# Sachin-A/TraceWeaver

Hardware: AMD Instinct MI355X
Metric: spans/sec reconstructed + assignment accuracy vs ground truth (higher is better)
Workload: dtype int64 timestamps, f64 scores; 1 GPU; media_microservices shape (6 services, E in {1,1,1,1,2,4}), 100000 requests/service x 16 replicas per GPU, concurrency 1.6, two-pass reconstruction, device mixture refit; spans_per_gpu=25600000, spans_total=25600000, parallelism=units sharded, 1 rank(s), backend none

## Files before the change

### traceweaver_amd/csrc/tw_engine.hip

```cpp
#include <algorithm>
#include <chrono>
#include <cmath>
#include <cstdio>
#include <cstdlib>
#include <cstring>
#include <functional>
#include <string>
#include <type_traits>
#include <vector>

#include <hip/hip_runtime.h>
#include <rocprim/rocprim.hpp>

#include "traceweaver_amd.h"
#include "tw_kernels.h"
#include "tw_fit.h"
#include "tw_eval.h"
#include "tw_skip.h"
#include "tw_load.h"
#include "tw_baselines.h"
#include "tw_stitch.h"
#include "tw_attr.h"
#include "tw_conf.h"
#include "tw_dist.h"
// ... 45 lines not shown

}

struct tw_engine {
    int device = 0;
    hipStream_t stream = nullptr;
    hipStream_t cls_stream[kMaxEp + 1] = {};
    hipEvent_t cls_ev[kMaxEp + 2] = {};
    hipStream_t sel_stream[3] = {};
    hipStream_t sel_stream2[3] = {};
    int64_t select_fork_min = 0;
    hipEvent_t prep_ev = nullptr;
    hipEvent_t post_fork[kMaxEp + 1] = {}, post_join[kMaxEp + 1][3] = {}, post_done[kMaxEp + 1] = {};
    hipEvent_t tile_ev[kMaxEp + 1] = {};
    hipStream_t cls_stream2[kMaxEp + 1] = {};
    hipEvent_t stretch_ev[kMaxEp + 1][kEnumStretches] = {}, stretch_done[kMaxEp + 1] = {};
    int enum_stretches = 1, stretch_min_tiles = 2048;
    int heavy_grid = 4096, select_grid = 0;
    int debug_lists = 0;
    int32_t first_lists[3][kMaxEp + 1] = {};
    hipEvent_t gate_ev = nullptr;
    int tile_gate = 0;
    int stage_min_tiles = 1024;
    int32_t *rank_in = nullptr, *rank_out = nullptr;
    bool class_params = false;
    int prio_min_e = 0, prio_high = 0;
    bool prio_any = false;
    int pipeline = 1;
    std::string err;
    int state = ST_EMPTY;
    int tile = kTile;
    int tile_threads = 2;
    int tile_single = 1;
    int tile_single_threads = 1;
    int coop = kCoop;
    std::vector<UnitDev> units;
    std::vector<TileDev> tiles;
    std::vector<int64_t> gs_off_h;
    std::vector<void*> allocs;
    void* arena = nullptr;
    size_t arena_cap = 0;
    bool arena_open = false;
    std::vector<std::pair<std::function<void(void*)>, size_t>> arena_req;
    Dev P{};
    int64_t n_ie = 0, n_gp = 0, n_slots = 0, n_gaps = 0;
    PairVI* agg_pair = nullptr;
    int32_t *agg_i32 = nullptr, *agg_i32b = nullptr;
    uint32_t *seg_in = nullptr, *seg_out = nullptr;
    int n_seg_out = 0;
    void* sort_tmp = nullptr;
    size_t sort_tmp_bytes = 0;
    double* mix_p_dev = nullptr;
    int32_t* mix_n_dev = nullptr;
    double* mix_c_dev = nullptr;
    double* gaps_sorted = nullptr;
    double* fit_models = nullptr;
    double* fit_uval = nullptr;
    int32_t *fit_ustart = nullptr, *fit_row_n = nullptr, *fit_row_uniq = nullptr;
    double* fit_centres = nullptr;
    double *fit_tape = nullptr, *fit_tape100 = nullptr;
    int64_t* fit_tape_off = nullptr;
    int64_t fit_tape_cap = 0;
    bool fit_runs_pending = false;
    bool fit_prepared = false;
    int tile_sub_max = 8;
    int32_t hard_pass1[kMaxEp + 1] = {};
    int8_t wide_pass1[kMaxEp + 1] = {};
    int32_t split_pass1[kMaxEp + 1] = {};
    int lean_pool = 512;
    bool pass1_done = false;
    std::vector<int32_t> fit_max_n;
    bool fit_max_n_valid = false;
    Mt19937 fit_rng;
    uint32_t fit_seed = 0;
    int32_t* slot_unit = nullptr;
    int32_t* tile_ids = nullptr;
    int32_t* ctr = nullptr;
    int64_t ctr_round_ints = 0, ctr_pass_ints = 0;
    int32_t tile_cls_off[kMaxEp + 2] = {};
    uint32_t *seg_gap = nullptr, *seg_gap_end = nullptr, *seg_gap_dst = nullptr;
    unsigned long long *comp_a = nullptr, *comp_b = nullptr;
    int64_t comp_cap = 0, n_gap_scored = 0;
    int32_t *truth = nullptr, *in_trace = nullptr;
    uint8_t* trace_bad = nullptr;
    unsigned long long* eval_counts = nullptr;
    int64_t n_traces = 0, trace_cap = 0;
    uint8_t* slot_scored = nullptr;
    int64_t n_gap_rows = 0;
    unsigned long long* key_acc = nullptr;
    double fit_ms = 0.0;
    int rounds = 0;
    bool skip_mode = false;
    SkipUnitDev* skip_units = nullptr;
    int32_t* skip_perm = nullptr; int64_t* skip_tw = nullptr; int32_t* skip_pool = nullptr; double* skip_dist = nullptr; long long* skip_fetch = nullptr;
    int64_t skip_fetch_n = 0;
    int64_t *orig_is = nullptr, *orig_ie = nullptr, *orig_os = nullptr, *orig_oe = nullptr;
    int32_t *orig_truth = nullptr, *orig_trace = nullptr;
    bool scaled_upload = false;
    hipEvent_t ev[EV_COUNT] = {};
    double ms[6] = {0, 0, 0, 0, 0, 0};
    StitchDev S{};
    int32_t* given_parent = nullptr;
    bool rows_set = false, parents_given = false, stitched = false;
    int64_t rows_cap = 0, st_trees = 0;
    int stitched_pass = -1;
    bool stitched_truth = false;
    AttrDev A{};
    bool groups_set = false, attributed = false;
    int64_t groups_cap = 0, attr_rows_cap = 0;
    ConfDev C{};
    int64_t conf_rows_cap = 0;
    DistDev D{};
// ... 183 lines not shown
    switch (code) {
        case TW_ERR_WINDOW_WIDTH: return "an incoming span has more candidate spans at one endpoint than the candidate bitmap holds";
        case TW_ERR_WINDOW_SIZE: return "a window holds more than TW_MAX_WINDOW incoming spans";
        case TW_ERR_NAN_PARAMS: return "a parameter block holds a single sample (std = NaN); the reference aborts here (n_in % 100 == 1)";
        case TW_ERR_SKIP_PARAMS: return "skip mode: the scorer needs a (mean, std) pair that BuildDistributions did not produce (the reference raises KeyError)";
        case TW_ERR_SKIP_REFERENCE_RAISES: return "skip mode: the reference raises on this input (all endpoints skipped, or a score tie compared through a skip span)";
        case TW_ERR_ARG: return "skip mode: a request starts before the first time window";
        default: return "kernel reported an error";
    }
}

template <class Tr>
int run_scan(tw_engine* e, const TileSet& S, hipStream_t st, typename Tr::T* agg) {
    const Dev& P = e->P;
    hipLaunchKernelGGL((k_scan_local<Tr>), dim3(S.n), dim3(e->tile), 0, st, P, S, agg);
    hipLaunchKernelGGL((k_scan_spine<Tr>), dim3(P.n_units), dim3(e->coop), 0, st, P, S, agg);
    hipLaunchKernelGGL((k_scan_fix<Tr>), dim3(S.n), dim3(e->tile), 0, st, P, S, agg);
    HIPCHK(hipGetLastError());
    return TW_OK;
}

TileSet all_tiles_host(const tw_engine* e) { return TileSet{nullptr, 0, e->P.n_tiles, 0}; }
TileSet class_tiles(const tw_engine* e, int E) { return TileSet{e->tile_ids + e->tile_cls_off[E], e->tile_cls_off[E], e->tile_cls_off[E + 1] - e->tile_cls_off[E], E}; }

int sort_ends(tw_engine* e, const TileSet& S, hipStream_t st) {
    const Dev& P = e->P;
    const dim3 tiles(S.n), tb(e->tile);
    hipLaunchKernelGGL(k_rank_ends, tiles, tb, 0, st, P, S, e->rank_in, e->rank_out);
    hipLaunchKernelGGL(k_place_ends, tiles, tb, 0, st, P, S, (const int32_t*)e->rank_in, (const int32_t*)e->rank_out);
    HIPCHK(hipGetLastError());
    return TW_OK;
}

int64_t part_extra(int cls, int64_t n_cls) {
    if (n_cls <= 0) return 0;
    static const int deep = env_int("TW_PART_BUDGET_DEEP", 2), shallow = env_int("TW_PART_BUDGET_SHALLOW", 0);
    if (cls <= 1) return 64;
    const int mult = cls >= 5 ? deep : shallow;
    return (mult > 0 ? n_cls * mult : n_cls / 8) + 64;
}

template <int E>
void launch_enumerate(tw_engine* e, int pass, int mode, const int32_t* listed) {
    const int nt = e->tile_cls_off[E + 1] - e->tile_cls_off[E];
    if (nt == 0) return;
    const int n_narrow = listed != nullptr ? listed[E] : -1, n_wide = listed != nullptr ? listed[kMaxEp + 1 + E] : ((pass == 2 && mode == 0 && e->wide_pass1[E] == 0) ? 0 : -1);
    if (n_narrow == 0 && n_wide == 0) return;
    hipStream_t st = e->cls_stream[E];
    (void)hipStreamWaitEvent(st, e->cls_ev[0], 0);
    if (mode == 0 && e->gate_ev != nullptr) (void)hipStreamWaitEvent(st, e->gate_ev, 0);
    const Dev& P = e->P;
    const dim3 hb(std::min(e->coop, kHeavyThreads));
    const int pool = E > 4 ? 2048 : (E > 1 ? kPairPoolPerEp * E : 1);
    const size_t pool_bytes = sizeof(double) * (size_t)pool;
    const size_t lean_bytes = sizeof(double) * (size_t)(2 * kMaxEp * kNarrow + e->lean_pool), lean_bytes_w = sizeof(double) * (size_t)(2 * kMaxEp * 64 * kCandWords + e->lean_pool);
    const bool lean = E >= P.lean_min_e && !e->skip_mode;
    const int cap = P.heavy_in_off[E + 1] - P.heavy_in_off[E];
    auto grid_for = [&](int known, int most) { return std::max(std::min(((known >= 0 ? known : cap) + kWorkChunk - 1) / kWorkChunk, most), 1); };
    auto narrow = [&](int part, int g) {
        if (lean) hipLaunchKernelGGL((k_enumerate_lean<kNarrow>), dim3(g), hb, lean_bytes, st, P, pass, mode, part, e->lean_pool, E, E);
        else hipLaunchKernelGGL((k_enumerate_heavy<E, kNarrow>), dim3(g), hb, pool_bytes, st, P, pass, mode, part, pool);
    };
    auto wide = [&](int part, int g) {
        if (lean) hipLaunchKernelGGL((k_enumerate_lean<64 * kCandWords>), dim3(g), hb, lean_bytes_w, st, P, pass, mode, part, e->lean_pool, E, E);
        else hipLaunchKernelGGL((k_enumerate_heavy<E, 64 * kCandWords>), dim3(g), hb, pool_bytes, st, P, pass, mode, part, pool);
    };
    bool stretched = false;
    if (mode == 0 && pass == 1 && e->class_params) {
        const TileSet S = class_tiles(e, E);
        (void)sort_ends(e, S, st);
        const int64_t total = e->n_gp;
        hipLaunchKernelGGL(k_block_params, dim3((unsigned)((total + 255) / 256)), dim3(256), 0, st, P, total, E);
    }
    if (mode == 0) {
        const bool single = E == 1 && e->tile_single != 0;
        const dim3 tile_block(e->tile >= 64 ? e->tile * (single ? e->tile_single_threads : e->tile_threads) : e->tile);
        int sub = 1;
        while (sub < e->tile_sub_max && nt * sub < 512 && (e->tile / (sub * 2)) * (sub * 2) == e->tile && e->tile / (sub * 2) >= 8) sub *= 2;
        const int ns = (!lean && !e->skip_mode && !(E >= 3 && E >= P.defer_min_e) && e->cls_stream2[E] != nullptr)
                           ? std::max(std::min(e->enum_stretches, nt / e->stretch_min_tiles), 1) : 1;
        stretched = ns > 1;
        for (int j = 0; j < ns; j++) {
            const int t0 = (int)((int64_t)nt * j / ns), t1 = (int)((int64_t)nt * (j + 1) / ns);
            const int32_t* ids = e->tile_ids + e->tile_cls_off[E] + t0;
            const bool sub_tile = e->tile == kTile && e->tile / sub == kSubTileSpans;
            if constexpr (E == 1) {
                if (single && sub_tile) hipLaunchKernelGGL((k_enumerate_tile<1, kSubTileSpans, true>), dim3((t1 - t0) * sub), tile_block, 0, st, P, pass, ids, t1 - t0, sub);
                else if (single) hipLaunchKernelGGL((k_enumerate_tile<1, kTile, true>), dim3((t1 - t0) * sub), tile_block, 0, st, P, pass, ids, t1 - t0, sub);
            }
            if (!single && sub_tile)
                hipLaunchKernelGGL((k_enumerate_tile<E, kSubTileSpans>), dim3((t1 - t0) * sub), tile_block, 0, st, P, pass, ids, t1 - t0, sub);
            else if (!single)
                hipLaunchKernelGGL((k_enumerate_tile<E>), dim3((t1 - t0) * sub), tile_block, 0, st, P, pass, ids, t1 - t0, sub);
            if (ns > 1) {
                hipLaunchKernelGGL(k_enum_snapshot, dim3(1), dim3(1), 0, st, P, E, j + 1);
                if (j + 1 < ns) {
                    hipStream_t s2 = e->cls_stream2[E];
                    (void)hipEventRecord(e->stretch_ev[E][j], st);
                    (void)hipStreamWaitEvent(s2, e->stretch_ev[E][j], 0);
                    hipLaunchKernelGGL((k_enumerate_heavy<E, kNarrow>), dim3(grid_for(-1, e->heavy_grid)), hb, pool_bytes, s2, P, pass, mode, (j + 1) << 8, pool);
                } else {
                    hipLaunchKernelGGL((k_enumerate_heavy<E, kNarrow>), dim3(grid_for(-1, e->heavy_grid)), hb, pool_bytes, st, P, pass, mode, (j + 1) << 8, pool);
                    (void)hipEventRecord(e->stretch_done[E], e->cls_stream2[E]);
                    (void)hipStreamWaitEvent(st, e->stretch_done[E], 0);
                }
// ... 187 lines not shown
    }
    const int bx = (int)std::min<int64_t>(std::max<int64_t>(4096 / nseg, 1), packed / nseg / 1024 + 1);
    const dim3 grid((unsigned)bx, (unsigned)std::min(nseg, 1024)), block(flat_threads(e));
    hipLaunchKernelGGL(k_rows_pack, grid, block, 0, e->stream, (const unsigned long long*)keys, seg_begin, seg_end, dst_off, nseg,
                       (int)begin_bit, (int)kb, e->comp_a);
    TWCHK(rocprim_call(e, [&](void* tmp, size_t& bytes) { return rocprim::radix_sort_keys(tmp, bytes, e->comp_a, e->comp_b, (size_t)packed, 0u, kb + segbits, e->stream); }));
    hipLaunchKernelGGL(k_rows_unpack, grid, block, 0, e->stream, (const unsigned long long*)e->comp_b, seg_begin, seg_end, dst_off, nseg,
                       (int)begin_bit, (int)kb, fixed, (unsigned long long*)out);
    HIPCHK(hipGetLastError());
    return TW_OK;
}

int run_pass(tw_engine* e, int pass) {
    const Dev& P = e->P;
    const dim3 tiles(P.n_tiles), tb(e->tile);
    const auto host_t0 = std::chrono::steady_clock::now();
    HIPCHK(hipEventRecord(e->ev[EV_BEGIN], e->stream));
    HIPCHK(hipMemsetAsync(e->ctr, 0, sizeof(int32_t) * (size_t)e->ctr_pass_ints, e->stream));
#ifdef TW_PROFILE
    HIPCHK(hipMemsetAsync(P.prof + 5, 0, sizeof(unsigned long long) * 3, e->stream));
    HIPCHK(hipMemsetAsync(P.prof + 10, 0, sizeof(unsigned long long) * 3, e->stream));
#endif
    int n_cls = 0;
    for (int E = 1; E <= kMaxEp; E++) n_cls += e->tile_cls_off[E + 1] > e->tile_cls_off[E] ? 1 : 0;
    const bool staged = !e->skip_mode && e->pipeline != 0 && P.n_tiles >= (int64_t)e->stage_min_tiles * std::max(n_cls, 1);
    e->class_params = false;
    if (pass == 1 && !e->skip_mode) {
        HIPCHK(hipMemsetAsync(e->rank_in, 0, sizeof(int32_t) * (size_t)std::max<int64_t>(P.n_in_total, 1), e->stream));
        HIPCHK(hipMemsetAsync(e->rank_out, 0, sizeof(int32_t) * (size_t)std::max<int64_t>(P.n_out_total, 1), e->stream));
        if (staged) e->class_params = true;
        else {
            int rc = sort_ends(e, all_tiles_host(e), e->stream);
            if (rc != TW_OK) return rc;
            const int64_t total = e->n_gp;
            hipLaunchKernelGGL(k_block_params, dim3((unsigned)((total + 255) / 256)), dim3(256), 0, e->stream, P, total, 0);
        }
    }
    if (e->skip_mode) {
        const int64_t total = e->n_gp;
        hipLaunchKernelGGL(k_neutral_params, dim3((unsigned)((total + 255) / 256)), dim3(256), 0, e->stream, P.gparam, total);
    }
    HIPCHK(hipEventRecord(e->ev[EV_PARAMS], e->stream));
    HIPCHK(hipEventRecord(e->ev[EV_ENUM0], e->stream));
    const auto host_t1 = std::chrono::steady_clock::now();
    {
        int rc = launch_enumerate_all(e, pass, 0, nullptr, staged, [&]() -> int {
            if (pass == 1) { int rs = run_scan<ScanMaxEnd>(e, all_tiles_host(e), e->stream, e->agg_pair); if (rs != TW_OK) return rs; }
            if (e->skip_mode) { HIPCHK(hipEventRecord(e->prep_ev, e->stream)); return TW_OK; }
            HIPCHK(hipMemsetAsync(P.w_conf, 0, sizeof(int32_t) * (size_t)P.n_in_total, e->stream));
            HIPCHK(hipMemsetAsync(P.gone_valid, 0, (size_t)P.n_in_total, e->stream));
            HIPCHK(hipMemsetAsync(P.w_dirty, 0, (size_t)P.n_in_total, e->stream));
            HIPCHK(hipMemsetAsync(P.owner, 0x7f, sizeof(int32_t) * std::max<int64_t>(P.n_out_total, 1), e->stream));
            HIPCHK(hipEventRecord(e->prep_ev, e->stream));
            return TW_OK;
        });
        if (rc != TW_OK) return rc;
    }
    e->host_ms[0] = std::chrono::duration<double, std::milli>(std::chrono::steady_clock::now() - host_t1).count();
    if (pass == 1 && !staged) {
        int rc = launch_windows(e, all_tiles_host(e), e->stream);
        if (rc != TW_OK) return rc;
    }
    if (!staged) HIPCHK(hipEventRecord(e->ev[EV_WIN], e->stream));
    if (e->skip_mode) {
        HIPCHK(hipMemsetAsync(P.owner, 0x7f, sizeof(int32_t) * std::max<int64_t>(P.n_out_total, 1), e->stream));
        HIPCHK(hipMemsetAsync(e->skip_fetch, 0, sizeof(long long) * (size_t)std::max<int64_t>(e->skip_fetch_n, 1), e->stream));
        HIPCHK(hipMemsetAsync(P.w_dirty, 0, (size_t)P.n_in_total, e->stream));
        hipLaunchKernelGGL(k_skip_walk, dim3(P.n_units), dim3(std::min(e->coop, 64)), 0, e->stream, P, (const SkipUnitDev*)e->skip_units);
// ... 181 lines not shown
        hipLaunchKernelGGL(k_load_local, dim3(side == 0 ? grid_in : grid_out), dim3(block), 0, e->stream, perm, row, (const uint32_t*)(side == 0 ? e->seg_in : e->seg_out), n);
        HIPCHK(hipGetLastError());
        int32_t* host = side == 0 ? in_perm : out_perm;
        if (host != nullptr) HIPCHK(hipMemcpyAsync(host, perm, sizeof(uint32_t) * n, hipMemcpyDeviceToHost, e->stream));
        HIPCHK(hipStreamSynchronize(e->stream));
    }
    hipLaunchKernelGGL(k_load_retruth, dim3(P.n_tiles), dim3(e->tile), 0, e->stream, L, (const int32_t*)pos_in, (const int32_t*)pos_out, e->truth,
                       has_trace ? e->in_trace : nullptr);
    HIPCHK(hipGetLastError());
    for (int u = 0; u < P.n_units; u++) {
        UnitDev& U = e->units[(size_t)u];
        U.tscale = std::ldexp(1.0, -kmax_h[(size_t)u]);
        U.float_time = 1;
        if (unit_time_scale != nullptr) unit_time_scale[u] = U.tscale;
    }
    HIPCHK(hipMemcpyAsync(const_cast<UnitDev*>(P.units), e->units.data(), sizeof(UnitDev) * e->units.size(), hipMemcpyHostToDevice, e->stream));
    HIPCHK(hipStreamSynchronize(e->stream));
    e->state = ST_LOADED; e->pass1_done = false;
    drop_batch_order(e);
    for (int E = 0; E <= kMaxEp; E++) { e->wide_pass1[E] = -1; e->hard_pass1[E] = -1; e->split_pass1[E] = -1; }
    return TW_OK;
}

extern "C" {

int tw_create(int device_id, tw_engine** out) {
    if (out == nullptr) return TW_ERR_ARG;
    *out = nullptr;
    tw_engine* e = new tw_engine();
    e->device = device_id;
    e->tile = std::min(std::max(env_int("TW_TILE", kTile), 1), kTile);
    e->tile_threads = std::min(std::max(env_int("TW_TILE_THREADS", 2), 1), 4);
    e->tile_single = env_int("TW_TILE_SINGLE", 1);
    e->tile_single_threads = std::min(std::max(env_int("TW_TILE_SINGLE_THREADS", 1), 1), 4);
    e->coop = std::min(std::max(env_int("TW_COOP_THREADS", kCoop), 1), kCoop);
    if (env_int("TW_SET_HW_QUEUES", 0) != 0) setenv("GPU_MAX_HW_QUEUES", "12", 0);
    hipError_t s = hipSetDevice(device_id);
    if (s == hipSuccess) s = hipStreamCreate(&e->stream);
    for (int i = 0; i < EV_COUNT && s == hipSuccess; i++) s = hipEventCreate(&e->ev[i]);
    for (int i = 0; i < SE_COUNT && s == hipSuccess; i++) s = hipEventCreate(&e->stage_ev[i]);
    const int prio_min_e = env_int("TW_PRIO_MIN_E", 0);
    int prio_least = 0, prio_greatest = 0;
    if (s == hipSuccess) s = hipDeviceGetStreamPriorityRange(&prio_least, &prio_greatest);
    e->prio_min_e = prio_min_e; e->prio_high = prio_greatest; e->prio_any = prio_greatest != prio_least;
    for (int i = 0; i <= kMaxEp + 1 && s == hipSuccess; i++) s = hipEventCreateWithFlags(&e->cls_ev[i], hipEventDisableTiming);
    if (s == hipSuccess) s = hipEventCreateWithFlags(&e->prep_ev, hipEventDisableTiming);
    for (int i = 0; i <= kMaxEp && s == hipSuccess; i++) {
        s = hipEventCreateWithFlags(&e->post_fork[i], hipEventDisableTiming);
        if (s == hipSuccess) s = hipEventCreateWithFlags(&e->tile_ev[i], hipEventDisableTiming);
        if (s == hipSuccess) s = hipEventCreateWithFlags(&e->post_done[i], hipEventDisableTiming);
        if (s == hipSuccess) s = hipEventCreateWithFlags(&e->stretch_done[i], hipEventDisableTiming);
        for (int j = 0; j < kEnumStretches && s == hipSuccess; j++) s = hipEventCreateWithFlags(&e->stretch_ev[i][j], hipEventDisableTiming);
        for (int j = 0; j < 3 && s == hipSuccess; j++) s = hipEventCreateWithFlags(&e->post_join[i][j], hipEventDisableTiming);
    }
    e->pipeline = env_int("TW_CLASS_PIPELINE", 1);
    e->sig_hash_bits = std::min(std::max(env_int("TW_SIG_HASH_BITS", 64), 1), 64);
    e->tile_gate = env_int("TW_TILE_GATE", 0);
    e->enum_stretches = std::min(std::max(env_int("TW_ENUM_STRETCHES", 1), 1), kEnumStretches);
    e->heavy_grid = std::max(env_int("TW_HEAVY_GRID", 4096), 64);
    e->select_grid = std::max(env_int("TW_SELECT_GRID", 0), 0);
    e->debug_lists = env_int("TW_DEBUG_LISTS", 0);
    e->select_fork_min = (int64_t)env_int("TW_SELECT_FORK_MIN", 0);
    e->stretch_min_tiles = std::max(env_int("TW_STRETCH_MIN_TILES", 2048), 1);
    e->stage_min_tiles = env_int("TW_STAGE_MIN_TILES", 1024);
    e->tile_sub_max = std::max(env_int("TW_TILE_SUB", 8), 1);
    e->lean_pool = std::min(std::max(env_int("TW_LEAN_POOL", 512), 1), 4096);
// ... 117 lines not shown
            U.key_rank[q] = (uint8_t)b->key_rank[epi + q];
            U.succ_mask[q] = sm;
            U.npred[q] = (uint8_t)np;
            std::stable_sort(U.pred_list[q], U.pred_list[q] + np, [&](uint8_t x, uint8_t y) {
                return b->key_rank[epi + x] < b->key_rank[epi + y];
            });
            for (int j = 0; j < np; j++) {
                const int p = U.pred_list[q][j];
                bool prim = true;
                for (int m = 0; m < E; m++)
                    if (m != p && m != q && dag[p * E + m] && dag[m * E + q]) prim = false;
                U.pred_prim[q][j] = prim ? 1 : 0;
            }
        }
        e->gs_off_h[(size_t)u] = gaps;
        ie += n * E;
        gp += (int64_t)U.nblk * U.nslot;
        slots += U.nslot;
        gaps += (int64_t)U.nslot * n;
        epi += E;
        dagi += E * E;
    }
    std::vector<int32_t> tile_ids_h;
    int32_t heavy_off_h[kMaxEp + 2] = {};
    for (int cls = 0; cls <= kMaxEp; cls++) {
        e->tile_cls_off[cls] = (int32_t)tile_ids_h.size();
        heavy_off_h[cls + 1] = heavy_off_h[cls];
        for (size_t tix = 0; tix < e->tiles.size(); tix++)
            if (e->units[(size_t)e->tiles[tix].unit].E == cls) tile_ids_h.push_back((int32_t)tix);
        for (int u = 0; u < b->n_units; u++)
            if (e->units[(size_t)u].E == cls) heavy_off_h[cls + 1] += e->units[(size_t)u].n_in;
    }
    e->tile_cls_off[kMaxEp + 1] = (int32_t)tile_ids_h.size();
    for (int cls = 1; cls <= kMaxEp; cls++)
        if (e->tile_cls_off[cls + 1] > e->tile_cls_off[cls]) {
            int rs = ensure_class_stream(e, cls); if (rs != TW_OK) return rs;
            if (e->enum_stretches > 1 && e->tile_cls_off[cls + 1] - e->tile_cls_off[cls] >= 2 * e->stretch_min_tiles && e->cls_stream2[cls] == nullptr)
                HIPCHK(hipStreamCreate(&e->cls_stream2[cls]));
        }
    for (int j = 0; j < 3; j++)
        if (e->sel_stream[j] == nullptr) HIPCHK(hipStreamCreate(&e->sel_stream[j]));
    {
        bool want = false;
        int deepest = 0;
        for (int cls = 1; cls <= kMaxEp; cls++) if (e->tile_cls_off[cls + 1] > e->tile_cls_off[cls]) deepest = cls;
        for (int cls = 1; cls < deepest; cls++) want |= e->select_fork_min > 0 && heavy_off_h[cls + 1] - heavy_off_h[cls] >= e->select_fork_min;
        for (int j = 0; j < 3 && want; j++)
            if (e->sel_stream2[j] == nullptr) HIPCHK(hipStreamCreate(&e->sel_stream2[j]));
    }
    const int64_t n_in_total = b->unit_in_off[b->n_units], n_out_total = b->ep_off[epi];
    if (n_in_total >= (1ll << 31) || n_out_total >= (1ll << 31)) return fail(e, TW_ERR_ARG, "batch exceeds 2^31 spans");
    if (gaps >= (1ll << 31)) return fail(e, TW_ERR_ARG, "batch too large: sum of nslot*n_in must stay below 2^31");
    std::vector<int32_t> slot_unit_h;
    std::vector<uint8_t> slot_scored_h;
    std::vector<uint32_t> seg_gap_h, seg_gap_end_h;
    for (int u = 0; u < b->n_units; u++) {
        const UnitDev& U = e->units[(size_t)u];
        const int E = U.E;
        for (int q = 0; q < U.nslot; q++) {
            bool scored;
            if (q < E) scored = U.npred[q] == 0;
            else if (q < E + E * E) {
                const int p = (q - E) / E, en = (q - E) % E;
                scored = false;
                for (int j = 0; j < U.npred[en]; j++) scored |= (U.pred_list[en][j] == p && U.pred_prim[en][j]);
            } else scored = true;
// ... 24 lines not shown
    P.batch_size = b->batch_size;
    P.batch_mis = b->batch_size_mis;
    P.split_twins = env_int("TW_SPLIT_TWINS", 2);
    P.defer_min_e = env_int("TW_DEFER_MIN_E", 5);
    P.lean_min_e = env_int("TW_LEAN_MIN_E", 5);
    P.lean_grid = std::max(env_int("TW_LEAN_GRID", TW_LEAN_GRID), 1);
    P.tile_max_deep = std::min(std::max(env_int("TW_TILE_MAX_DEEP", kTileMax), 0), kTileMax);
    int rc;
    e->arena_req.clear();
    e->arena_open = true;
    UnitDev* d_units; TileDev* d_tiles; int64_t *d_is, *d_ie, *d_os, *d_oe, *d_gs;
    DEV_ALLOC(d_units, P.n_units); DEV_ALLOC(d_tiles, P.n_tiles);
    DEV_ALLOC(d_is, n_in_total); DEV_ALLOC(d_ie, n_in_total); DEV_ALLOC(d_os, n_out_total); DEV_ALLOC(d_oe, n_out_total);
    DEV_ALLOC(d_gs, P.n_units);
    DEV_ALLOC(P.in_end_sorted, n_in_total); DEV_ALLOC(P.out_end_sorted, n_out_total);
    DEV_ALLOC(P.gparam, gp * 4);
    DEV_ALLOC(e->mix_n_dev, slots); DEV_ALLOC(e->mix_p_dev, slots * kMaxComp * 3); DEV_ALLOC(e->mix_c_dev, slots * kMaxComp * 4);
    DEV_ALLOC(P.pm_val, n_in_total); DEV_ALLOC(P.pm_idx, n_in_total); DEV_ALLOC(P.pc, n_in_total + 1); DEV_ALLOC(P.seg, n_in_total);
    DEV_ALLOC(P.win_end, n_in_total); DEV_ALLOC(P.wid, n_in_total); DEV_ALLOC(P.w_last, n_in_total);
    DEV_ALLOC(P.unit_nwin, P.n_units); DEV_ALLOC(P.w_dirty, n_in_total); DEV_ALLOC(P.w_conf, n_in_total);
    DEV_ALLOC(P.tk_n, n_in_total); DEV_ALLOC(P.leaves, n_in_total); DEV_ALLOC(P.leaves0, n_in_total); DEV_ALLOC(P.chosen, n_in_total); DEV_ALLOC(P.rep, n_in_total);
    DEV_ALLOC(P.tkr_n, n_in_total);
    DEV_ALLOC(P.tk_idx, ie * kTopK); DEV_ALLOC(P.tkr_idx, ie * kTopK);
    DEV_ALLOC(P.tk_score, n_in_total * kTopK); DEV_ALLOC(P.tkr_score, n_in_total * kTopK);
    DEV_ALLOC(P.c_lo, ie); DEV_ALLOC(P.c_hi, ie); DEV_ALLOC(P.c_bits, ie * kCandWords); DEV_ALLOC(P.parent, ie);
    DEV_ALLOC(P.gone, ie * kCandWords); DEV_ALLOC(P.gone_valid, n_in_total); DEV_ALLOC(P.leaves_r, n_in_total);
    DEV_ALLOC(P.frontier, (int64_t)kFrontierSlots * 2 * kFrontierCap); 
    P.frontier_big_slots = (int32_t)std::min<int64_t>(std::max<int64_t>(n_in_total / 16384, kFrontierBigSlots), std::max(kFrontierBigSlots, 512));
    DEV_ALLOC(P.frontier_big, (int64_t)P.frontier_big_slots * 2 * kFrontierBigCap);
    DEV_ALLOC(P.pair_pool, (int64_t)kPairSlots * kPairSpill);
    DEV_ALLOC(P.owner, n_out_total);
    DEV_ALLOC(P.gaps, gaps);
    DEV_ALLOC(e->tile_ids, (int64_t)tile_ids_h.size());
    DEV_ALLOC(P.heavy_in_unit, n_in_total); DEV_ALLOC(P.heavy_in_idx, n_in_total);
    {
        int64_t big_total = 0, slots = 0, want = 0;
        for (int cls = 0; cls <= kMaxEp; cls++) want += 2 * part_extra(cls, heavy_off_h[cls + 1] - heavy_off_h[cls]);
        static const int64_t slots_max = (int64_t)std::max(env_int("TW_PART_SLOTS_MAX", 16 << 20), 1024);
        for (int cls = 0; cls <= kMaxEp; cls++) {
            const int64_t n_cls = heavy_off_h[cls + 1] - heavy_off_h[cls];
            int64_t extra = part_extra(cls, n_cls);
            if (want > slots_max && extra > 64) extra = std::max<int64_t>((int64_t)((double)extra * (double)slots_max / (double)want), std::min<int64_t>(n_cls / 8 + 64, extra));
            P.heavy_big_off[cls] = (int32_t)big_total; P.part_off[cls] = (int32_t)slots;
            big_total += n_cls + extra; slots += 2 * extra;
        }
        P.heavy_big_off[kMaxEp + 1] = (int32_t)big_total; P.part_off[kMaxEp + 1] = (int32_t)slots;
        DEV_ALLOC(P.heavy_big_unit, big_total); DEV_ALLOC(P.heavy_big_idx, big_total);
        DEV_ALLOC(P.heavy_big_part, big_total); DEV_ALLOC(P.heavy_big_slot, big_total);
        DEV_ALLOC(P.fb_unit, big_total); DEV_ALLOC(P.fb_idx, big_total); DEV_ALLOC(P.fb_part, big_total); DEV_ALLOC(P.fb_slot, big_total);
        DEV_ALLOC(P.split_unit, slots); DEV_ALLOC(P.split_idx, slots); DEV_ALLOC(P.split_slot, slots); DEV_ALLOC(P.split_parts, slots);
        DEV_ALLOC(P.part_n, slots); DEV_ALLOC(P.part_leaves, slots); DEV_ALLOC(P.part_score, slots * kTopK); DEV_ALLOC(P.part_idx, slots * kTopK * kMaxEp);
        DEV_ALLOC(P.part_bits, slots * kMaxEp * kCandWords);
        DEV_ALLOC(P.part_logn, slots); DEV_ALLOC(P.part_log_sc, slots * kPartLogCap); DEV_ALLOC(P.part_log_ix, slots * kPartLogCap);
        DEV_ALLOC(P.part_lo, slots); DEV_ALLOC(P.part_hi, slots); DEV_ALLOC(P.part_lvl, slots);
        int64_t deep = 0;
        for (int cls = std::max(P.defer_min_e, 3); cls <= kMaxEp; cls++) deep += heavy_off_h[cls + 1] - heavy_off_h[cls];
        P.defer_cap = (int32_t)(deep > 0 ? std::min<int64_t>(std::max<int64_t>(deep * kDeferListPerSpan, kDeferListMin), 1ll << 28) : 1);
        DEV_ALLOC(P.defer_list, P.defer_cap);
    }
    for (int cls = 0; cls <= kMaxEp + 1; cls++) P.heavy_in_off[cls] = heavy_off_h[cls];
    DEV_ALLOC(P.prof, 32); DEV_ALLOC(e->key_acc, 2);
    const int64_t sel_cap = (int64_t)P.n_tiles * e->tile + 1;
    {
        int64_t at = 0;
        auto take = [&](int64_t ints) { const int64_t o = at; at += (ints + 31) / 32 * 32; return o; };
        const int64_t o_hc = take(kSelSlots * 4 * kSelSeg * kCtrStride), o_hn = take(kSelSlots * 8), o_ic = take(2 * (kMaxEp + 1)), o_in = take(8 * (kMaxEp + 1)), o_bc = take(kMaxEp + 1),
// ... 65 lines not shown
    if (rc != TW_OK) return rc;
    if (e->skip_mode) {
        for (int u = 0; u < b->n_units; u++) {
            SkipUnitDev K{};
            K.perm = e->skip_perm; K.tw_start = e->skip_tw + sk_tw_off[(size_t)u]; K.pool = e->skip_pool + sk_pool_off[(size_t)u];
            K.dist = e->skip_dist + sk_dist_off[(size_t)u]; K.fetches = e->skip_fetch + sk_pool_off[(size_t)u]; K.n_tw = b->skip[u].n_tw;
            skip_h.push_back(K);
        }
        HIPCHK(hipMemcpyAsync(e->skip_units, skip_h.data(), sizeof(SkipUnitDev) * skip_h.size(), hipMemcpyHostToDevice, e->stream));
        HIPCHK(hipMemcpyAsync(e->skip_perm, perm_h.data(), sizeof(int32_t) * perm_h.size(), hipMemcpyHostToDevice, e->stream));
        HIPCHK(hipMemcpyAsync(e->skip_tw, tw_h.data(), sizeof(int64_t) * tw_h.size(), hipMemcpyHostToDevice, e->stream));
        HIPCHK(hipMemcpyAsync(e->skip_pool, pool_h.data(), sizeof(int32_t) * pool_h.size(), hipMemcpyHostToDevice, e->stream));
        HIPCHK(hipMemcpyAsync(e->skip_dist, dist_h.data(), sizeof(double) * dist_h.size(), hipMemcpyHostToDevice, e->stream));
        HIPCHK(hipStreamSynchronize(e->stream));
    }
    HIPCHK(hipMemsetAsync(P.prof, 0, sizeof(unsigned long long) * 32, e->stream));
    HIPCHK(hipMemsetAsync(P.prof + 10, 0xff, sizeof(unsigned long long), e->stream));
    P.units = d_units; P.tiles = d_tiles;
    P.in_start = d_is; P.in_end = d_ie; P.out_start = d_os; P.out_end = d_oe;
    P.gs_off = d_gs;
    P.mix_n = e->mix_n_dev; P.mix_c = e->mix_c_dev;
    e->sort_tmp = nullptr; e->sort_tmp_bytes = 0;
    const hipMemcpyKind kind = spans_on_device ? hipMemcpyDeviceToDevice : hipMemcpyHostToDevice;
    HIPCHK(hipMemcpyAsync(d_is, b->in_start, sizeof(int64_t) * n_in_total, kind, e->stream));
    HIPCHK(hipMemcpyAsync(d_ie, b->in_end, sizeof(int64_t) * n_in_total, kind, e->stream));
    HIPCHK(hipMemcpyAsync(d_os, b->out_start, sizeof(int64_t) * n_out_total, kind, e->stream));
    HIPCHK(hipMemcpyAsync(d_oe, b->out_end, sizeof(int64_t) * n_out_total, kind, e->stream));
    HIPCHK(hipMemcpyAsync(d_units, e->units.data(), sizeof(UnitDev) * e->units.size(), hipMemcpyHostToDevice, e->stream));
    HIPCHK(hipMemcpyAsync(d_tiles, e->tiles.data(), sizeof(TileDev) * e->tiles.size(), hipMemcpyHostToDevice, e->stream));
    HIPCHK(hipMemcpyAsync(d_gs, e->gs_off_h.data(), sizeof(int64_t) * e->gs_off_h.size(), hipMemcpyHostToDevice, e->stream));
    HIPCHK(hipMemcpyAsync(e->seg_in, seg_in.data(), sizeof(uint32_t) * seg_in.size(), hipMemcpyHostToDevice, e->stream));
    HIPCHK(hipMemcpyAsync(e->seg_out, seg_out.data(), sizeof(uint32_t) * seg_out.size(), hipMemcpyHostToDevice, e->stream));
    HIPCHK(hipMemcpyAsync(e->tile_ids, tile_ids_h.data(), sizeof(int32_t) * tile_ids_h.size(), hipMemcpyHostToDevice, e->stream));
    HIPCHK(hipMemcpyAsync(e->slot_unit, slot_unit_h.data(), sizeof(int32_t) * slot_unit_h.size(), hipMemcpyHostToDevice, e->stream));
    HIPCHK(hipMemcpyAsync(e->seg_gap, seg_gap_h.data(), sizeof(uint32_t) * seg_gap_h.size(), hipMemcpyHostToDevice, e->stream));
    HIPCHK(hipMemcpyAsync(e->seg_gap_end, seg_gap_end_h.data(), sizeof(uint32_t) * seg_gap_end_h.size(), hipMemcpyHostToDevice, e->stream));
    HIPCHK(hipMemcpyAsync(e->seg_gap_dst, seg_gap_dst_h.data(), sizeof(uint32_t) * seg_gap_dst_h.size(), hipMemcpyHostToDevice, e->stream));
    HIPCHK(hipMemcpyAsync(e->slot_scored, slot_scored_h.data(), slot_scored_h.size(), hipMemcpyHostToDevice, e->stream));
    HIPCHK(hipMemsetAsync(P.gaps, 0xff, sizeof(double) * std::max<int64_t>(gaps, 1), e->stream));
    HIPCHK(hipMemsetAsync(P.pc, 0, (size_t)n_in_total + 1, e->stream));
    HIPCHK(hipMemsetAsync(P.tk_idx, 0xff, sizeof(int32_t) * (size_t)std::max<int64_t>(ie * kTopK, 1), e->stream));
    HIPCHK(hipMemsetAsync(P.tk_score, 0xff, sizeof(double) * (size_t)std::max<int64_t>(n_in_total * kTopK, 1), e->stream));
    HIPCHK(hipMemsetAsync(e->mix_n_dev, 0, sizeof(int32_t) * std::max<int64_t>(slots, 1), e->stream));
    HIPCHK(hipStreamSynchronize(e->stream));
    e->scaled_upload = b->unit_time_scale != nullptr;
    e->state = ST_LOADED; e->pass1_done = false;
    for (int E = 0; E <= kMaxEp; E++) { e->wide_pass1[E] = -1; e->hard_pass1[E] = -1; e->split_pass1[E] = -1; }
    return TW_OK;
}

int tw_run_pass1(tw_engine* e) {
    if (e == nullptr) return TW_ERR_ARG;
    if (e->state < ST_LOADED) return fail(e, TW_ERR_STATE, "tw_run_pass1 before tw_load_batch");
    HIPCHK(hipSetDevice(e->device));
    drop_forest(e);
    const int rc = run_pass(e, 1);
    e->fit_prepared = false; e->fit_runs_pending = false; e->fit_max_n_valid = false;
    if (rc == TW_OK) { e->state = ST_PASS1; e->pass1_done = true; }
    return rc;
}

int tw_get_gaps(tw_engine* e, double* gaps) {
    if (e == nullptr || gaps == nullptr) return TW_ERR_ARG;
    if (e->state != ST_PASS1) return fail(e, TW_ERR_STATE, "tw_get_gaps is valid right after tw_run_pass1");
    if (e->skip_mode) return fail(e, TW_ERR_STATE, "a skip-mode batch runs one pass (traceweaver_v3.py:1155-1156): there is no refit");
    HIPCHK(hipSetDevice(e->device));
// ... 1643 lines not shown
```

### traceweaver_amd/csrc/tw_kernels.h

```cpp
#pragma once
#include "tw_device.h"

namespace tw {

__device__ __forceinline__ void raise_err(const Dev& P, int code) { atomicCAS(P.err, 0, code); }

__device__ __forceinline__ int wave_append(int32_t* counter, bool pred, int lane_in = -1) {
    const unsigned long long mask = __ballot(pred);
    if (mask == 0) return -1;
    const int lane = lane_in >= 0 ? lane_in : (int)(threadIdx.x & 63), leader = __ffsll((long long)mask) - 1;
    int base = 0;
    if (lane == leader) base = atomicAdd(counter, __popcll(mask));
#ifndef TW_HOST_EMULATION
    if (lane_in >= 0) base = __builtin_amdgcn_readlane(base, leader);
    else
#endif
    base = __shfl(base, leader);
    return pred ? base + __popcll(mask & ((1ull << lane) - 1ull)) : -1;
}
__device__ __forceinline__ int bump_reserve(int32_t* counter, int n, int budget) {
    if (atomicAdd(counter, 0) + n > budget) return -1;
    const int old = atomicAdd(counter, n);
    return old + n <= budget ? old : -1;
}
// ... 102 lines not shown
            out[i] = fixed | ((comp[d + (i - a)] & mask) << begin_bit);
    }
}

__device__ __forceinline__ int set_tile(const TileSet& S) { return S.ids != nullptr ? S.ids[blockIdx.x] : (int)blockIdx.x; }
__device__ __forceinline__ TileSet all_tiles(const Dev& P) { return TileSet{nullptr, 0, P.n_tiles, 0}; }

__device__ __forceinline__ void rank_list(const int64_t* st, const int64_t* en, int n, int i, int32_t* delta) {
    const int64_t a = en[i];
    int cnt = 0;
    for (int j = i + 1; j < n && st[j] < a; j++)
        if (en[j] < a) { cnt++; atomicAdd(&delta[j], -1); }
    if (cnt) atomicAdd(&delta[i], cnt);
}
__global__ void k_rank_ends(Dev P, TileSet S, int32_t* d_in, int32_t* d_out) {
    const TileDev Tl = P.tiles[set_tile(S)];
    const UnitDev& U = P.units[Tl.unit];
    const int i = Tl.first + threadIdx.x;
    if (i >= U.n_in) return;
    rank_list(P.in_start + U.in_off, P.in_end + U.in_off, U.n_in, i, d_in + U.in_off);
    for (int e = 0; e < U.E; e++)
        rank_list(P.out_start + U.ep_off[e], P.out_end + U.ep_off[e], (int)(U.ep_off[e + 1] - U.ep_off[e]), i, d_out + U.ep_off[e]);
}
__global__ void k_place_ends(Dev P, TileSet S, const int32_t* d_in, const int32_t* d_out) {
    const TileDev Tl = P.tiles[set_tile(S)];
    const UnitDev& U = P.units[Tl.unit];
    const int i = Tl.first + threadIdx.x;
    if (i >= U.n_in) return;
    P.in_end_sorted[U.in_off + i + d_in[U.in_off + i]] = P.in_end[U.in_off + i];
    for (int e = 0; e < U.E; e++)
        P.out_end_sorted[U.ep_off[e] + i + d_out[U.ep_off[e] + i]] = P.out_end[U.ep_off[e] + i];
}

__global__ void k_block_params(Dev P, int64_t total, int cls) {
    const int64_t g = (int64_t)blockIdx.x * blockDim.x + threadIdx.x;
    if (g >= total) return;
    int lo = 0, hi = P.n_units - 1;
    while (lo < hi) {
        const int mid = (lo + hi + 1) >> 1;
        if (P.units[mid].gp_off <= g) lo = mid; else hi = mid - 1;
    }
    const UnitDev& U = P.units[lo];
    if (cls > 0 && U.E != cls) return;
    const int64_t r = g - U.gp_off;
    const int b = (int)(r / U.nslot), q = (int)(r % U.nslot), E = U.E;
    double* out = P.gparam + g * 4;
    const int64_t *t1 = nullptr, *t2 = nullptr;
    if (q < E) {
        if (U.npred[q] == 0) { t1 = P.in_start + U.in_off; t2 = P.out_start + U.ep_off[q]; }
    } else if (q < E + E * E) {
        const int p = (q - E) / E, e = (q - E) % E;
        bool prim = false;
        for (int j = 0; j < U.npred[e]; j++) prim |= (U.pred_list[e][j] == p && U.pred_prim[e][j]);
        if (prim) { t1 = P.out_end_sorted + U.ep_off[p]; t2 = P.out_start + U.ep_off[e]; }
    } else {
        const int e = q - E - E * E;
        t1 = P.out_end_sorted + U.ep_off[e];
        t2 = P.in_end_sorted + U.in_off;
    }
    if (t1 == nullptr) { out[0] = out[1] = out[2] = out[3] = dnan(); return; }
    const int a = b * P.batch_size, z = min(a + P.batch_size, U.n_in), len = z - a;
    double bm[10], mean;
    const int bs = (len + 9) / 10;
    int m = 0;
    if (!U.float_time) {
        int64_t s1 = 0, s2 = 0;
        for (int kb = 0; kb < 10; kb++) {
            const int st = kb * bs, en = min((kb + 1) * bs, len);
            if (en - st <= 0) continue;
            int64_t u1 = 0, u2 = 0;
            for (int i = a + st; i < a + en; i++) { u1 += t1[i]; u2 += t2[i]; }
            s1 += u1; s2 += u2;
            bm[m++] = (double)(u2 - u1) / (double)(en - st);
        }
        mean = (double)(s2 - s1) / (double)len;
    } else {
        double s1 = 0.0, s2 = 0.0;
        for (int kb = 0; kb < 10; kb++) {
            const int st = kb * bs, en = min((kb + 1) * bs, len);
            if (en - st <= 0) continue;
            double u1 = 0.0, u2 = 0.0;
            for (int i = a + st; i < a + en; i++) {
                const double v1 = (double)t1[i], v2 = (double)t2[i];
                u1 += v1; u2 += v2; s1 += v1; s2 += v2;
            }
            bm[m++] = (u2 - u1) / (double)(en - st);
        }
        mean = (s2 - s1) / (double)len;
    }
    const double mu = np_sum(bm, m) / (double)m;
    double d2[10];
    for (int kb = 0; kb < m; kb++) { const double d = bm[kb] - mu; d2[kb] = d * d; }
    const double var = np_sum(d2, m) / (double)(m - 1);
    const double sd = (sqrt((double)bs) * sqrt(var)) * U.tscale;
    if (sd != sd) raise_err(P, TW_ERR_NAN_PARAMS);
    const double used = sd < 1.0e-12 ? 0.001 : sd;
    out[0] = mean; out[1] = sd; out[2] = tw_log(used); out[3] = used / U.tscale;
}

__global__ void k_mix_consts(const double* mix_p, const int32_t* mix_n, const int32_t* slot_unit, const UnitDev* units, double* mix_c, int64_t total) {
    const int64_t g = (int64_t)blockIdx.x * blockDim.x + threadIdx.x;
    if (g >= total) return;
    const int64_t slot = g / kMaxComp;
    const double tscale = units[slot_unit[slot]].tscale;
    if (mix_n[slot] <= 0) {
        if (g % kMaxComp == 0) { mix_c[g * 4 + 0] = 0.0; mix_c[g * 4 + 1] = 0.001 / tscale; mix_c[g * 4 + 2] = tw_log(0.001); mix_c[g * 4 + 3] = 0.0; }
        return;
    }
    const double w = mix_p[g * 3 + 0], mu = mix_p[g * 3 + 1], pc = mix_p[g * 3 + 2];
    mix_c[g * 4 + 0] = mu * pc; mix_c[g * 4 + 1] = pc * tscale; mix_c[g * 4 + 2] = tw_log(pc); mix_c[g * 4 + 3] = tw_log(w);
}

struct Scorer {
    int pass;
    const double* gp;
    const int32_t* mix_n;
    const double* mix_c;
};

__device__ __forceinline__ double term_gauss(double mean, double used, double logstd, double x) {
    const double y = (x - mean) / used;
    return (-(y * y) / 2.0 - kLogSqrt2Pi) - logstd;
}

__device__ __forceinline__ double term_mix_inline(int n, const double* c, double x) {
    double a0 = 0.0, a1 = 0.0, a2 = 0.0, a3 = 0.0, a4 = 0.0, amax = -dinf();
    for (int k = 0; k < n; k++) {
        const double y = x * c[k * 4 + 1] - c[k * 4 + 0];
        const double lp = y * y;
        const double ak = (-0.5 * (kLog2Pi + lp) + c[k * 4 + 2]) + c[k * 4 + 3];
// ... 3079 lines not shown
```

Before: 1.322 billion spans/s.

## Compute per-batch parameter sums once per wavefront with shared-memory atomics

Adds a wavefront-per-block-group kernel that reads each timestamp array once per batch. It accumulates the ten sub-block sums in LDS with atomics, then lets lanes finish every slot's mean and standard deviation from those shared sums. Before, one thread per slot re-scanned both arrays for its slot, and every class launch swept all slots with a binary search. A precomputed host table of (unit, block) groups per class replaces that sweep. The trade-off is contended 64-bit shared atomics and lanes that have little work on small batches.

```diff
diff --git a/traceweaver_amd/csrc/tw_engine.hip b/traceweaver_amd/csrc/tw_engine.hip
--- a/traceweaver_amd/csrc/tw_engine.hip
+++ b/traceweaver_amd/csrc/tw_engine.hip
@@ -101,6 +101,7 @@
     int tile = kTile;
     int tile_threads = 2;
     int tile_single = 1;
+    int block_params = 1;
     int tile_single_threads = 1;
     int coop = kCoop;
     std::vector<UnitDev> units;
@@ -147,6 +148,8 @@
     int32_t* ctr = nullptr;
     int64_t ctr_round_ints = 0, ctr_pass_ints = 0;
     int32_t tile_cls_off[kMaxEp + 2] = {};
+    BlockRef* blk_tab = nullptr;
+    int32_t blk_cls_off[kMaxEp + 2] = {};
     uint32_t *seg_gap = nullptr, *seg_gap_end = nullptr, *seg_gap_dst = nullptr;
     unsigned long long *comp_a = nullptr, *comp_b = nullptr;
     int64_t comp_cap = 0, n_gap_scored = 0;
@@ -396,6 +399,19 @@
     return TW_OK;
 }
 
+void launch_block_params(tw_engine* e, int cls, hipStream_t st) {
+    const Dev& P = e->P;
+    if (e->block_params == 0) {
+        const int64_t total = e->n_gp;
+        hipLaunchKernelGGL(k_block_params, dim3((unsigned)((total + 255) / 256)), dim3(256), 0, st, P, total, cls);
+        return;
+    }
+    const int n = e->blk_cls_off[cls + 1] - e->blk_cls_off[cls];
+    if (n <= 0) return;
+    const int threads = e->coop >= 64 ? 64 * std::min(e->coop / 64, kParamWaves) : e->coop, waves = std::max(threads / 64, 1);
+    hipLaunchKernelGGL(k_block_params_wave, dim3((unsigned)((n + waves - 1) / waves)), dim3(threads), 0, st, P, (const BlockRef*)(e->blk_tab + e->blk_cls_off[cls]), n);
+}
+
 int64_t part_extra(int cls, int64_t n_cls) {
     if (n_cls <= 0) return 0;
     static const int deep = env_int("TW_PART_BUDGET_DEEP", 2), shallow = env_int("TW_PART_BUDGET_SHALLOW", 0);
@@ -433,8 +449,7 @@
     if (mode == 0 && pass == 1 && e->class_params) {
         const TileSet S = class_tiles(e, E);
         (void)sort_ends(e, S, st);
-        const int64_t total = e->n_gp;
-        hipLaunchKernelGGL(k_block_params, dim3((unsigned)((total + 255) / 256)), dim3(256), 0, st, P, total, E);
+        launch_block_params(e, E, st);
     }
     if (mode == 0) {
         const bool single = E == 1 && e->tile_single != 0;
@@ -688,8 +703,7 @@
         else {
             int rc = sort_ends(e, all_tiles_host(e), e->stream);
             if (rc != TW_OK) return rc;
-            const int64_t total = e->n_gp;
-            hipLaunchKernelGGL(k_block_params, dim3((unsigned)((total + 255) / 256)), dim3(256), 0, e->stream, P, total, 0);
+            launch_block_params(e, 0, e->stream);
         }
     }
     if (e->skip_mode) {
@@ -937,6 +951,7 @@
     e->tile = std::min(std::max(env_int("TW_TILE", kTile), 1), kTile);
     e->tile_threads = std::min(std::max(env_int("TW_TILE_THREADS", 2), 1), 4);
     e->tile_single = env_int("TW_TILE_SINGLE", 1);
+    e->block_params = env_int("TW_BLOCK_PARAMS", 1);
     e->tile_single_threads = std::min(std::max(env_int("TW_TILE_SINGLE_THREADS", 1), 1), 4);
     e->coop = std::min(std::max(env_int("TW_COOP_THREADS", kCoop), 1), kCoop);
     if (env_int("TW_SET_HW_QUEUES", 0) != 0) setenv("GPU_MAX_HW_QUEUES", "12", 0);
@@ -1120,6 +1135,14 @@
             if (e->units[(size_t)u].E == cls) heavy_off_h[cls + 1] += e->units[(size_t)u].n_in;
     }
     e->tile_cls_off[kMaxEp + 1] = (int32_t)tile_ids_h.size();
+    std::vector<BlockRef> blk_tab_h;
+    for (int cls = 0; cls <= kMaxEp; cls++) {
+        e->blk_cls_off[cls] = (int32_t)blk_tab_h.size();
+        for (int u = 0; u < b->n_units; u++)
+            if (cls == 0 || e->units[(size_t)u].E == cls)
+                for (int k = 0; k < e->units[(size_t)u].nblk; k += param_group(e->units[(size_t)u].E)) blk_tab_h.push_back(BlockRef{u, k});
+    }
+    e->blk_cls_off[kMaxEp + 1] = (int32_t)blk_tab_h.size();
     for (int cls = 1; cls <= kMaxEp; cls++)
         if (e->tile_cls_off[cls + 1] > e->tile_cls_off[cls]) {
             int rs = ensure_class_stream(e, cls); if (rs != TW_OK) return rs;
@@ -1210,6 +1233,7 @@
     DEV_ALLOC(P.owner, n_out_total);
     DEV_ALLOC(P.gaps, gaps);
     DEV_ALLOC(e->tile_ids, (int64_t)tile_ids_h.size());
+    DEV_ALLOC(e->blk_tab, (int64_t)blk_tab_h.size());
     DEV_ALLOC(P.heavy_in_unit, n_in_total); DEV_ALLOC(P.heavy_in_idx, n_in_total);
     {
         int64_t big_total = 0, slots = 0, want = 0;
@@ -1341,6 +1365,7 @@
     HIPCHK(hipMemcpyAsync(e->seg_in, seg_in.data(), sizeof(uint32_t) * seg_in.size(), hipMemcpyHostToDevice, e->stream));
     HIPCHK(hipMemcpyAsync(e->seg_out, seg_out.data(), sizeof(uint32_t) * seg_out.size(), hipMemcpyHostToDevice, e->stream));
     HIPCHK(hipMemcpyAsync(e->tile_ids, tile_ids_h.data(), sizeof(int32_t) * tile_ids_h.size(), hipMemcpyHostToDevice, e->stream));
+    HIPCHK(hipMemcpyAsync(e->blk_tab, blk_tab_h.data(), sizeof(BlockRef) * blk_tab_h.size(), hipMemcpyHostToDevice, e->stream));
     HIPCHK(hipMemcpyAsync(e->slot_unit, slot_unit_h.data(), sizeof(int32_t) * slot_unit_h.size(), hipMemcpyHostToDevice, e->stream));
     HIPCHK(hipMemcpyAsync(e->seg_gap, seg_gap_h.data(), sizeof(uint32_t) * seg_gap_h.size(), hipMemcpyHostToDevice, e->stream));
     HIPCHK(hipMemcpyAsync(e->seg_gap_end, seg_gap_end_h.data(), sizeof(uint32_t) * seg_gap_end_h.size(), hipMemcpyHostToDevice, e->stream));
diff --git a/traceweaver_amd/csrc/tw_kernels.h b/traceweaver_amd/csrc/tw_kernels.h
--- a/traceweaver_amd/csrc/tw_kernels.h
+++ b/traceweaver_amd/csrc/tw_kernels.h
@@ -158,6 +158,45 @@
         P.out_end_sorted[U.ep_off[e] + i + d_out[U.ep_off[e] + i]] = P.out_end[U.ep_off[e] + i];
 }
 
+constexpr int kParamArrays = 2 + 2 * kMaxEp;
+__device__ __forceinline__ const int64_t* param_array(const Dev& P, const UnitDev& U, int id) {
+    if (id < 2) return (id == 0 ? P.in_start : P.in_end_sorted) + U.in_off;
+    return ((id & 1) ? P.out_end_sorted : P.out_start) + U.ep_off[(id - 2) >> 1];
+}
+__device__ __forceinline__ bool param_slot(const UnitDev& U, int q, int& a1, int& a2) {
+    const int E = U.E;
+    if (q < E) {
+        a1 = 0; a2 = 2 + 2 * q;
+        return U.npred[q] == 0;
+    }
+    if (q < E + E * E) {
+        const int p = (q - E) / E, e = (q - E) % E;
+        bool prim = false;
+        for (int j = 0; j < U.npred[e]; j++) prim |= (U.pred_list[e][j] == p && U.pred_prim[e][j]);
+        a1 = 3 + 2 * p; a2 = 2 + 2 * e;
+        return prim;
+    }
+    a1 = 3 + 2 * (q - E - E * E); a2 = 1;
+    return true;
+}
+__device__ __forceinline__ int param_sums_float(const int64_t* t1, const int64_t* t2, int a, int len, int bs, double* bm, double& mean) {
+    double s1 = 0.0, s2 = 0.0;
+    int m = 0;
+    for (int kb = 0; kb < 10; kb++) {
+        const int st = kb * bs, en = min((kb + 1) * bs, len);
+        if (en - st <= 0) continue;
+        double u1 = 0.0, u2 = 0.0;
+        for (int i = a + st; i < a + en; i++) {
+            const double v1 = (double)t1[i], v2 = (double)t2[i];
+            u1 += v1; u2 += v2; s1 += v1; s2 += v2;
+        }
+        bm[m++] = (u2 - u1) / (double)(en - st);
+    }
+    mean = (s2 - s1) / (double)len;
+    return m;
+}
+__device__ __forceinline__ void param_finish(const Dev& P, const UnitDev& U, const double* bm, int m, int bs, double mean, double* out);
+
 __global__ void k_block_params(Dev P, int64_t total, int cls) {
     const int64_t g = (int64_t)blockIdx.x * blockDim.x + threadIdx.x;
     if (g >= total) return;
@@ -169,22 +208,11 @@
     const UnitDev& U = P.units[lo];
     if (cls > 0 && U.E != cls) return;
     const int64_t r = g - U.gp_off;
-    const int b = (int)(r / U.nslot), q = (int)(r % U.nslot), E = U.E;
+    const int b = (int)(r / U.nslot), q = (int)(r % U.nslot);
     double* out = P.gparam + g * 4;
-    const int64_t *t1 = nullptr, *t2 = nullptr;
-    if (q < E) {
-        if (U.npred[q] == 0) { t1 = P.in_start + U.in_off; t2 = P.out_start + U.ep_off[q]; }
-    } else if (q < E + E * E) {
-        const int p = (q - E) / E, e = (q - E) % E;
-        bool prim = false;
-        for (int j = 0; j < U.npred[e]; j++) prim |= (U.pred_list[e][j] == p && U.pred_prim[e][j]);
-        if (prim) { t1 = P.out_end_sorted + U.ep_off[p]; t2 = P.out_start + U.ep_off[e]; }
-    } else {
-        const int e = q - E - E * E;
-        t1 = P.out_end_sorted + U.ep_off[e];
-        t2 = P.in_end_sorted + U.in_off;
-    }
-    if (t1 == nullptr) { out[0] = out[1] = out[2] = out[3] = dnan(); return; }
+    int a1, a2;
+    if (!param_slot(U, q, a1, a2)) { out[0] = out[1] = out[2] = out[3] = dnan(); return; }
+    const int64_t *t1 = param_array(P, U, a1), *t2 = param_array(P, U, a2);
     const int a = b * P.batch_size, z = min(a + P.batch_size, U.n_in), len = z - a;
     double bm[10], mean;
     const int bs = (len + 9) / 10;
@@ -200,20 +228,11 @@
             bm[m++] = (double)(u2 - u1) / (double)(en - st);
         }
         mean = (double)(s2 - s1) / (double)len;
-    } else {
-        double s1 = 0.0, s2 = 0.0;
-        for (int kb = 0; kb < 10; kb++) {
-            const int st = kb * bs, en = min((kb + 1) * bs, len);
-            if (en - st <= 0) continue;
-            double u1 = 0.0, u2 = 0.0;
-            for (int i = a + st; i < a + en; i++) {
-                const double v1 = (double)t1[i], v2 = (double)t2[i];
-                u1 += v1; u2 += v2; s1 += v1; s2 += v2;
-            }
-            bm[m++] = (u2 - u1) / (double)(en - st);
-        }
-        mean = (s2 - s1) / (double)len;
-    }
+    } else m = param_sums_float(t1, t2, a, len, bs, bm, mean);
+    param_finish(P, U, bm, m, bs, mean, out);
+}
+
+__device__ __forceinline__ void param_finish(const Dev& P, const UnitDev& U, const double* bm, int m, int bs, double mean, double* out) {
     const double mu = np_sum(bm, m) / (double)m;
     double d2[10];
     for (int kb = 0; kb < m; kb++) { const double d = bm[kb] - mu; d2[kb] = d * d; }
@@ -222,6 +241,90 @@
     if (sd != sd) raise_err(P, TW_ERR_NAN_PARAMS);
     const double used = sd < 1.0e-12 ? 0.001 : sd;
     out[0] = mean; out[1] = sd; out[2] = tw_log(used); out[3] = used / U.tscale;
+}
+
+constexpr int kParamWaves = 4;
+constexpr int kParamSums = 256;
+static_assert(kParamArrays * 10 <= kParamSums, "a block's sums fit the wavefront's table");
+static_assert(kMaxEp * kMaxEp + 2 * kMaxEp <= 128, "a lane finishes at most two slots");
+__host__ __device__ inline int param_group(int E) {
+    const int by_lanes = 64 / (E * E + 2 * E), by_sums = kParamSums / ((2 + 2 * E) * 10), g = by_lanes < by_sums ? by_lanes : by_sums;
+    return g > 1 ? g : 1;
+}
+struct BlockRef {
+    int32_t unit, blk;
+};
+
+__device__ __forceinline__ void param_slot_finish(const Dev& P, const UnitDev& U, const unsigned long long* sum, int q, int a, int len, int bs, double* out) {
+    int a1, a2;
+    if (!param_slot(U, q, a1, a2)) { out[0] = out[1] = out[2] = out[3] = dnan(); return; }
+    double bm[10], mean;
+    int m = 0;
+    if (!U.float_time) {
+        int64_t s1 = 0, s2 = 0;
+        for (int kb = 0; kb < 10; kb++) {
+            const int st = kb * bs, en = min((kb + 1) * bs, len);
+            if (en - st <= 0) continue;
+            const int64_t u1 = (int64_t)sum[a1 * 10 + kb], u2 = (int64_t)sum[a2 * 10 + kb];
+            s1 += u1; s2 += u2;
+            bm[m++] = (double)(u2 - u1) / (double)(en - st);
+        }
+        mean = (double)(s2 - s1) / (double)len;
+    } else m = param_sums_float(param_array(P, U, a1), param_array(P, U, a2), a, len, bs, bm, mean);
+    param_finish(P, U, bm, m, bs, mean, out);
+}
+__device__ __forceinline__ void param_group_finish(const Dev& P, const UnitDev& U, const unsigned long long* sum, int blk0, int t) {
+    const int g = t / U.nslot, q = t - g * U.nslot;
+    const int a = (blk0 + g) * P.batch_size, len = min(a + P.batch_size, U.n_in) - a;
+    param_slot_finish(P, U, sum + g * (2 + 2 * U.E) * 10, q, a, len, (len + 9) / 10, P.gparam + (U.gp_off + (int64_t)(blk0 + g) * U.nslot + q) * 4);
+}
+
+template <int N>
+__device__ __forceinline__ void param_add_spans(const Dev& P, const UnitDev& U, int E, int i, unsigned long long* sum) {
+    if (E != N) {
+        if constexpr (N < kMaxEp) param_add_spans<N + 1>(P, U, E, i, sum);
+        return;
+    }
+    int64_t v[2 * (N + 1)];
+#pragma unroll
+    for (int p = 0; p <= N; p++) {
+        const int64_t at = (p == 0 ? U.in_off : U.ep_off[p == 0 ? 0 : p - 1]) + i;
+        v[2 * p] = (p == 0 ? P.in_start : P.out_start)[at];
+        v[2 * p + 1] = (p == 0 ? P.in_end_sorted : P.out_end_sorted)[at];
+    }
+#pragma unroll
+    for (int p = 0; p <= N; p++) {
+        atomicAdd(&sum[(2 * p) * 10], (unsigned long long)v[2 * p]);
+        atomicAdd(&sum[(2 * p + 1) * 10], (unsigned long long)v[2 * p + 1]);
+    }
+}
+
+__global__ void __launch_bounds__(64 * kParamWaves) k_block_params_wave(Dev P, const BlockRef* groups, int n_groups) {
+    __shared__ unsigned long long sh_sum[kParamWaves][kParamSums];
+    const int W = min((int)blockDim.x, 64), wave = (int)threadIdx.x / 64, lane = (int)threadIdx.x % 64;
+    const int64_t item = (int64_t)blockIdx.x * (blockDim.x >= 64 ? blockDim.x / 64 : 1) + wave;
+    if (wave >= kParamWaves || item >= n_groups) return;
+    const int unit = __builtin_amdgcn_readfirstlane(groups[item].unit), blk0 = __builtin_amdgcn_readfirstlane(groups[item].blk);
+    const UnitDev& U = P.units[unit];
+    const int E = U.E, na = 2 + 2 * E, nb = min(param_group(E), U.nblk - blk0);
+    unsigned long long* sum = sh_sum[wave];
+    if (!U.float_time) {
+        for (int k = lane; k < nb * na * 10; k += W) sum[k] = 0ull;
+        wave_sync();
+        for (int g = 0; g < nb; g++) {
+            const int a = (blk0 + g) * P.batch_size, len = min(a + P.batch_size, U.n_in) - a, bs = (len + 9) / 10;
+            for (int i = lane; i < len; i += W)
+                param_add_spans<1>(P, U, E, a + i, sum + g * na * 10 + i / bs);
+        }
+        wave_sync();
+    }
+    const int n_fin = nb * U.nslot;
+#ifdef TW_HOST_EMULATION
+    for (int t = lane; t < n_fin; t += W) param_group_finish(P, U, sum, blk0, t);
+#else
+    if (lane < n_fin) param_group_finish(P, U, sum, blk0, lane);
+    if (lane + 64 < n_fin) param_group_finish(P, U, sum, blk0, lane + 64);
+#endif
 }
 
 __global__ void k_mix_consts(const double* mix_p, const int32_t* mix_n, const int32_t* slot_unit, const UnitDev* units, double* mix_c, int64_t total) {
```

Result: faster. 1.338 billion spans/s (median of 6 runs) (+1.2%).
